# HiLab-git/FPL-plus

Hardware: AMD Instinct MI355X
Metric: 3D volumes/sec (train step, 80x160x160) (higher is better)
Workload: dtype bf16; 1 GPU; UNet3D-DSBN 32-base-ch bf16 (fp32 master weights), per-GPU batch 2x1x80x160x160 synthetic VS crops, DiceLoss + Adam, domain alternating per step; global_batch=2, parallelism=dp1, step=zero_grad+forward+loss+backward+allreduce+adam

## Files before the change

### fpl-plus_amd/csrc/elementwise.hip

```cpp
#include "common.h"
#include "philox.h"

namespace {

constexpr int EW_THREADS = 256;

template <typename T> struct Vec;
template <> struct Vec<float> {
  static constexpr int N = 4;
  typedef float4 raw;
  static __device__ __forceinline__ void load(const float* p, float (&v)[4]) {
    const float4 r = *reinterpret_cast<const float4*>(p);
    v[0] = r.x; v[1] = r.y; v[2] = r.z; v[3] = r.w;
  }
  static __device__ __forceinline__ void load_nt(const float* p, float (&v)[4]) { load(p, v); }
  static __device__ __forceinline__ void store(float* p, const float (&v)[4]) {
    *reinterpret_cast<float4*>(p) = make_float4(v[0], v[1], v[2], v[3]);
  }
};
template <> struct Vec<bf16_t> {
  static constexpr int N = 8;
  typedef __attribute__((ext_vector_type(8))) __bf16 raw;
  static __device__ __forceinline__ void load(const bf16_t* p, float (&v)[8]) {
    const raw r = *reinterpret_cast<const raw*>(p);
// ... 563 lines not shown
      vis[t] = ((n * D + pd * d_o + (t >> 2)) * H + 2 * ho + ((t >> 1) & 1)) * W + 2 * wo + (t & 1);
      ldv_nt<T, VEC>(y + vis[t] * ldy + c0, a[t]);
    }
#pragma unroll
    for (int j = 0; j < VEC; ++j) best[j] = -INFINITY;
#pragma unroll
    for (int t = 0; t < 8; ++t) {
      if (t >= 4 * pd) break;
#pragma unroll
      for (int j = 0; j < VEC; ++j) {
        float z = fmaf(a[t][j], sc[j], sh[j]);
        z = z > 0.f ? z : z * slope;
        z = (float)(T)z;
        a[t][j] = z;
        best[j] = z > best[j] ? z : best[j];
      }
      stv<T, VEC>(out + vis[t] * ldo + c0, a[t]);
    }
    stv<T, VEC>(pooled + vo * ldp + c0, best);
  }
}

template <typename T, int VEC>
__global__ void __launch_bounds__(EW_THREADS)
pool_bwd_bn_reduce_k(const T* __restrict__ y, int64_t ldy, const T* __restrict__ dy, int64_t lddy, const T* __restrict__ dskip,
                     int64_t lds, T* __restrict__ dx, int64_t ldo, const float* __restrict__ mean,
                     const float* __restrict__ rstd, const float* __restrict__ scale, const float* __restrict__ shift,
                     const float* __restrict__ slope_p, int N, int D, int H, int W, int C, int pd, float* __restrict__ part) {
  const int G = C / VEC, VL = EW_THREADS / G;
  const int g = threadIdx.x % G, vl = threadIdx.x / G, c0 = g * VEC;
  const int Do = D / pd, Ho = H / 2, Wo = W / 2;
  const int64_t vout = (int64_t)N * Do * Ho * Wo;
  const float slope = *slope_p;
  float sdz[VEC], sdx[VEC], sds = 0.f, m[VEC], rs[VEC], sc[VEC], sh[VEC];
#pragma unroll
  for (int j = 0; j < VEC; ++j) {
    sdz[j] = sdx[j] = 0.f;
    m[j] = mean[c0 + j]; rs[j] = rstd[c0 + j]; sc[j] = scale[c0 + j]; sh[j] = shift[c0 + j];
  }
  for (int64_t vo = (int64_t)blockIdx.x * VL + vl; vo < vout; vo += (int64_t)gridDim.x * VL) {
    int64_t q = vo;
    const int wo = (int)(q % Wo); q /= Wo;
    const int ho = (int)(q % Ho); q /= Ho;
    const int d_o = (int)(q % Do);
    const int64_t n = q / Do;
    float gr[VEC], best[VEC], a[8][VEC], o[8][VEC];
    int arg[VEC];
    int64_t vis[8];
    ldv<T, VEC>(dy + vo * lddy + c0, gr);
#pragma unroll
    for (int t = 0; t < 8; ++t) {
      if (t >= 4 * pd) break;
      vis[t] = ((n * D + pd * d_o + (t >> 2)) * H + 2 * ho + ((t >> 1) & 1)) * W + 2 * wo + (t & 1);
      ldv<T, VEC>(y + vis[t] * ldy + c0, a[t]);
      if (dskip) ldv<T, VEC>(dskip + vis[t] * lds + c0, o[t]);
      else {
#pragma unroll
        for (int j = 0; j < VEC; ++j) o[t][j] = 0.f;
      }
    }
#pragma unroll
    for (int j = 0; j < VEC; ++j) { best[j] = -INFINITY; arg[j] = 0; }
#pragma unroll
    for (int t = 0; t < 8; ++t) {
      if (t >= 4 * pd) break;
#pragma unroll
      for (int j = 0; j < VEC; ++j) {
        float z = fmaf(a[t][j], sc[j], sh[j]);
        z = z > 0.f ? z : z * slope;
        z = (float)(T)z;
        if (z > best[j]) { best[j] = z; arg[j] = t; }
      }
    }
#pragma unroll
    for (int t = 0; t < 8; ++t) {
      if (t >= 4 * pd) break;
#pragma unroll
      for (int j = 0; j < VEC; ++j) {
        const float dv = (float)(T)(o[t][j] + ((arg[j] == t) ? gr[j] : 0.f));
        o[t][j] = dv;
        const float z = fmaf(a[t][j], sc[j], sh[j]);
        const float dz = z > 0.f ? dv : dv * slope;
        sds += z > 0.f ? 0.f : dv * z;
        sdz[j] += dz;
        sdx[j] = fmaf(dz, (a[t][j] - m[j]) * rs[j], sdx[j]);
      }
      stv<T, VEC>(dx + vis[t] * ldo + c0, o[t]);
    }
  }
  __shared__ float red[EW_THREADS / 64 * 64][2 * VEC + 1];
  float* row = part + (int64_t)blockIdx.x * (2 * C + 1);
  for (int ofs = G; ofs < 64; ofs <<= 1) {
#pragma unroll
    for (int j = 0; j < VEC; ++j) { sdz[j] += __shfl_xor(sdz[j], ofs, 64); sdx[j] += __shfl_xor(sdx[j], ofs, 64); }
    sds += __shfl_xor(sds, ofs, 64);
  }
  const int lane = threadIdx.x & 63, wave = threadIdx.x >> 6;
  if (lane < G) {
#pragma unroll
    for (int j = 0; j < VEC; ++j) { red[wave * 64 + lane][j] = sdz[j]; red[wave * 64 + lane][VEC + j] = sdx[j]; }
    red[wave * 64 + lane][2 * VEC] = sds;
  }
  __syncthreads();
  if ((int)threadIdx.x < G) {
#pragma unroll
    for (int j = 0; j < VEC; ++j) {
      float t0 = 0.f, t1 = 0.f;
#pragma unroll
      for (int wv = 0; wv < EW_THREADS / 64; ++wv) { t0 += red[wv * 64 + threadIdx.x][j]; t1 += red[wv * 64 + threadIdx.x][VEC + j]; }
      row[c0 + j] = t0;
// ... 40 lines not shown
#pragma unroll
    for (int t = 0; t < 4; ++t) {
      if (t >= 2 * pd) break;
#pragma unroll
      for (int j = 0; j < VEC; ++j) {
        float z = fmaf(a[t][j], sc[j], sh[j]);
        z = z > 0.f ? z : z * slope;
        z = (float)(T)z;
        a[t][j] = z;
        best[j] = z > best[j] ? z : best[j];
      }
      stv<T, VEC>(out + vis[t] * ldo + c0, a[t]);
    }
#pragma unroll
    for (int j = 0; j < VEC; ++j) {
      const float o = __shfl_xor(best[j], G, 64);
      best[j] = o > best[j] ? o : best[j];
    }
    if (!(w & 1)) stv<T, VEC>(pooled + (int64_t)(u >> 1) * ldp + c0, best);
  }
}

template <typename T, int VEC>
__global__ void __launch_bounds__(EW_THREADS)
pool_bwd_bn_reduce_col_k(const T* __restrict__ y, int64_t ldy, const T* __restrict__ dy, int64_t lddy,
                         const T* __restrict__ dskip, int64_t lds, T* __restrict__ dx, int64_t ldo,
                         const float* __restrict__ mean, const float* __restrict__ rstd, const float* __restrict__ scale,
                         const float* __restrict__ shift, const float* __restrict__ slope_p, int N, int D, int H, int W, int C,
                         int pd, float* __restrict__ part) {
  const int G = C / VEC, VL = EW_THREADS / G;
  const int g = threadIdx.x % G, vl = threadIdx.x / G, c0 = g * VEC;
  const int Do = D / pd, Ho = H / 2;
  const unsigned units = (unsigned)N * Do * Ho * W;
  const float slope = *slope_p;
  float sdz[VEC], sdx[VEC], sds = 0.f, m[VEC], rs[VEC], sc[VEC], sh[VEC];
#pragma unroll
  for (int j = 0; j < VEC; ++j) {
    sdz[j] = sdx[j] = 0.f;
    m[j] = mean[c0 + j]; rs[j] = rstd[c0 + j]; sc[j] = scale[c0 + j]; sh[j] = shift[c0 + j];
  }
  for (unsigned u = blockIdx.x * VL + vl; u < units; u += gridDim.x * VL) {
    unsigned q = u;
    const int w = (int)(q % (unsigned)W); q /= (unsigned)W;
    const int ho = (int)(q % (unsigned)Ho); q /= (unsigned)Ho;
    const int d_o = (int)(q % (unsigned)Do);
    const int64_t n = q / (unsigned)Do;
    float gr[VEC], best[VEC], a[4][VEC], o[4][VEC];
    int arg[VEC];
    int64_t vis[4];
    ldv<T, VEC>(dy + (int64_t)(u >> 1) * lddy + c0, gr);
#pragma unroll
    for (int t = 0; t < 4; ++t) {
      if (t >= 2 * pd) break;
      vis[t] = ((n * D + pd * d_o + (t >> 1)) * H + 2 * ho + (t & 1)) * W + w;
      ldv<T, VEC>(y + vis[t] * ldy + c0, a[t]);
      if (dskip) ldv<T, VEC>(dskip + vis[t] * lds + c0, o[t]);
      else {
#pragma unroll
        for (int j = 0; j < VEC; ++j) o[t][j] = 0.f;
      }
    }
#pragma unroll
    for (int j = 0; j < VEC; ++j) { best[j] = -INFINITY; arg[j] = 8; }
#pragma unroll
    for (int t = 0; t < 4; ++t) {
      if (t >= 2 * pd) break;
#pragma unroll
      for (int j = 0; j < VEC; ++j) {
        float z = fmaf(a[t][j], sc[j], sh[j]);
        z = z > 0.f ? z : z * slope;
        z = (float)(T)z;
        if (z > best[j]) { best[j] = z; arg[j] = 2 * t + (w & 1); }
      }
    }
#pragma unroll
    for (int j = 0; j < VEC; ++j) {
      const float ob = __shfl_xor(best[j], G, 64);
      const int oa = __shfl_xor(arg[j], G, 64);
      if (ob > best[j] || (ob == best[j] && oa < arg[j])) arg[j] = -1;
    }
#pragma unroll
    for (int t = 0; t < 4; ++t) {
      if (t >= 2 * pd) break;
#pragma unroll
      for (int j = 0; j < VEC; ++j) {
        const float dv = (float)(T)(o[t][j] + ((arg[j] == 2 * t + (w & 1)) ? gr[j] : 0.f));
        o[t][j] = dv;
        const float z = fmaf(a[t][j], sc[j], sh[j]);
        const float dz = z > 0.f ? dv : dv * slope;
        sds += z > 0.f ? 0.f : dv * z;
        sdz[j] += dz;
        sdx[j] = fmaf(dz, (a[t][j] - m[j]) * rs[j], sdx[j]);
      }
      stv<T, VEC>(dx + vis[t] * ldo + c0, o[t]);
    }
  }
  __shared__ float red[EW_THREADS / 64 * 64][2 * VEC + 1];
  float* row = part + (int64_t)blockIdx.x * (2 * C + 1);
  for (int ofs = G; ofs < 64; ofs <<= 1) {
#pragma unroll
    for (int j = 0; j < VEC; ++j) { sdz[j] += __shfl_xor(sdz[j], ofs, 64); sdx[j] += __shfl_xor(sdx[j], ofs, 64); }
    sds += __shfl_xor(sds, ofs, 64);
  }
  const int lane = threadIdx.x & 63, wave = threadIdx.x >> 6;
  if (lane < G) {
#pragma unroll
    for (int j = 0; j < VEC; ++j) { red[wave * 64 + lane][j] = sdz[j]; red[wave * 64 + lane][VEC + j] = sdx[j]; }
    red[wave * 64 + lane][2 * VEC] = sds;
  }
  __syncthreads();
  if ((int)threadIdx.x < G) {
#pragma unroll
    for (int j = 0; j < VEC; ++j) {
      float t0 = 0.f, t1 = 0.f;
#pragma unroll
      for (int wv = 0; wv < EW_THREADS / 64; ++wv) { t0 += red[wv * 64 + threadIdx.x][j]; t1 += red[wv * 64 + threadIdx.x][VEC + j]; }
      row[c0 + j] = t0;
      row[C + c0 + j] = t1;
    }
  }
  if (threadIdx.x == 0) {
    float t = 0.f;
    for (int wv = 0; wv < EW_THREADS / 64; ++wv)
      for (int k = 0; k < G; ++k) t += red[wv * 64 + k][2 * VEC];
    row[2 * C] = t;
  }
}

__global__ void __launch_bounds__(EW_THREADS)
adam_k(float* __restrict__ p, const float* __restrict__ g, float* __restrict__ m, float* __restrict__ v, int64_t n,
       float step_size, float b1, float b2, float eps, float wd, float inv_sqrt_bc2, float gscale) {
  const FplxAdamConst c = {step_size, b1, b2, eps, wd, inv_sqrt_bc2, gscale, 1.f - b1, 1.f - b2};
  for (int64_t i = (int64_t)blockIdx.x * EW_THREADS + threadIdx.x; i < n; i += (int64_t)gridDim.x * EW_THREADS) {
    float pi = p[i], mi = m[i], vi = v[i];
    fplx_adam_elem(pi, g[i], mi, vi, c);
    m[i] = mi;
    v[i] = vi;
    p[i] = pi;
  }
}


template <typename T>
__global__ void __launch_bounds__(EW_THREADS)
channel_stats_k(const T* __restrict__ x, int64_t ld, int64_t V, int C, float* __restrict__ part) {
  const int c = blockIdx.y * 64 + (threadIdx.x & 63);
  const int vl = threadIdx.x >> 6;
  float s = 0.f, q = 0.f;
// ... 251 lines not shown
  FPLX_REQUIRE(n > 0 && c > 0 && d >= pd && h >= 2 && w >= 2 && !(d % pd) && !(h & 1) && !(w & 1) && (pd == 1 || pd == 2),
               FPLX_E_BADSHAPE, "%s: bad shape", what);
  FPLX_REQUIRE(fplx_bn_pool_fused_ok(c, dt), FPLX_E_BADSHAPE, "%s: C=%d dtype %d not supported (fplx_bn_pool_fused_ok)", what, c, dt);
  return FPLX_OK;
}

int fplx_bn_act_pool_fwd(const void* y, int64_t ldy, void* out, int64_t ldo, void* pooled, int64_t ldp, const float* scale,
                         const float* shift, const float* slope, int n, int d, int h, int w, int c, int dt, int pd,
                         fplx_stream_t stream) {
  FPLX_REQUIRE(y && out && pooled && scale && shift && slope, FPLX_E_NULL, "bn_act_pool_fwd: null pointer");
  const int rc = bn_pool_args_ok("bn_act_pool_fwd", n, d, h, w, c, dt, pd);
  if (rc != FPLX_OK) return rc;
  FPLX_REQUIRE(vec_ok<bf16_t>(y, ldy, out, ldo, pooled, ldp, c), FPLX_E_BADSHAPE, "bn_act_pool_fwd: pointers / leading dimensions not 16-byte aligned");
  const int64_t vo = (int64_t)n * (d / pd) * (h / 2) * (w / 2);
  if (fplx_knob(FPLX_K_POOL_COL) && c / 8 <= 32 && 2 * vo < ((int64_t)1 << 31))
    bn_act_pool_fwd_col_k<bf16_t, 8><<<ew_grid(2 * vo * (c / 8)), EW_THREADS, 0, (hipStream_t)stream>>>(
        (const bf16_t*)y, ldy, (bf16_t*)out, ldo, (bf16_t*)pooled, ldp, scale, shift, slope, n, d, h, w, c, pd);
  else
  bn_act_pool_fwd_k<bf16_t, 8><<<ew_grid(vo * (c / 8)), EW_THREADS, 0, (hipStream_t)stream>>>(
      (const bf16_t*)y, ldy, (bf16_t*)out, ldo, (bf16_t*)pooled, ldp, scale, shift, slope, n, d, h, w, c, pd);
  return fplx_check_launch("bn_act_pool_fwd");
}

int fplx_pool_bwd_bn_reduce(const void* y, int64_t ldy, const void* dy, int64_t lddy, const void* dskip, int64_t lds, void* dx,
                            int64_t ldo, const float* mean, const float* rstd, const float* scale, const float* shift,
                            const float* slope, int n, int d, int h, int w, int c, int dt, int pd, float* part,
                            fplx_stream_t stream) {
  FPLX_REQUIRE(y && dy && dx && mean && rstd && scale && shift && slope && part, FPLX_E_NULL, "pool_bwd_bn_reduce: null pointer");
  const int rc = bn_pool_args_ok("pool_bwd_bn_reduce", n, d, h, w, c, dt, pd);
  if (rc != FPLX_OK) return rc;
  FPLX_REQUIRE(vec_ok<bf16_t>(y, ldy, dy, lddy, dx, ldo, c) && vec_ok<bf16_t>(dskip, lds, nullptr, 0, nullptr, 0, c), FPLX_E_BADSHAPE,
               "pool_bwd_bn_reduce: pointers / leading dimensions not 16-byte aligned");
  const int rows = fplx_rows_for((int64_t)n * d * h * w);
  if (fplx_knob(FPLX_K_POOL_COL) && c / 8 <= 32 && (int64_t)n * (d / pd) * (h / 2) * w < ((int64_t)1 << 31))
    pool_bwd_bn_reduce_col_k<bf16_t, 8><<<rows, EW_THREADS, 0, (hipStream_t)stream>>>(
        (const bf16_t*)y, ldy, (const bf16_t*)dy, lddy, (const bf16_t*)dskip, lds, (bf16_t*)dx, ldo, mean, rstd, scale, shift, slope, n,
        d, h, w, c, pd, part);
  else
  pool_bwd_bn_reduce_k<bf16_t, 8><<<rows, EW_THREADS, 0, (hipStream_t)stream>>>(
      (const bf16_t*)y, ldy, (const bf16_t*)dy, lddy, (const bf16_t*)dskip, lds, (bf16_t*)dx, ldo, mean, rstd, scale, shift, slope, n,
      d, h, w, c, pd, part);
  return fplx_check_launch("pool_bwd_bn_reduce");
}

int fplx_adam_step(float* p, const float* g, float* m, float* v, int64_t n, float lr, float beta1, float beta2,
                   float eps, float weight_decay, int step, float grad_scale, fplx_stream_t stream) {
  FPLX_REQUIRE(p && g && m && v, FPLX_E_NULL, "adam_step: null pointer");
  FPLX_REQUIRE(n > 0 && step >= 1, FPLX_E_BADSHAPE, "adam_step: n=%lld step=%d", (long long)n, step);
  const double bc1 = 1.0 - pow((double)beta1, step), bc2 = 1.0 - pow((double)beta2, step);
  adam_k<<<ew_grid(n), EW_THREADS, 0, (hipStream_t)stream>>>(p, g, m, v, n, (float)((double)lr / bc1), beta1, beta2, eps,
                                                            weight_decay, (float)(1.0 / sqrt(bc2)), grad_scale);
  return fplx_check_launch("adam_step");
}

}
```

### fpl-plus_amd/fplx/_lib.py

```python
import ctypes
import os
import re

_RUNTIME_ENV = (("GPU_MAX_HW_QUEUES", "8"), ("HIP_FORCE_DEV_KERNARG", "1"))
_env_preset = {k: os.environ.get(k) for k, _ in _RUNTIME_ENV}
for _k, _v in _RUNTIME_ENV:
    os.environ.setdefault(_k, _v)

import torch


def runtime_env_report():
    return dict(_env_report)


_gpu_was_up = bool(torch.cuda.is_initialized())
_env_report = {}
for _k, _v in _RUNTIME_ENV:
    _env_report[_k] = (os.environ.get(_k), "preset" if _env_preset[_k] is not None else ("too late" if _gpu_was_up else "fplx"))
_late = [k for k, (_, how) in _env_report.items() if how == "too late"]
if _late:
    import warnings
    warnings.warn(
        "fplx was imported after the GPU had been initialised and %s %s not in the environment: the HIP runtime reads %s only "
# ... 98 lines not shown
    try:
        while _lib.fplx_tuning_key(i, buf, 64) >= 0:
            key = buf.value.decode()
            env = os.environ.get("FPLX_" + key.upper())
            if env is not None:
                try:
                    val = int(env)
                except ValueError:
                    raise ValueError("fplx: FPLX_%s=%r is not an integer" % (key.upper(), env))
                rc = _lib.fplx_set_tuning(key.encode(), val)
                if rc != 0:
                    raise FplxError("fplx (%d): fplx_set_tuning(%s, %d) failed" % (rc, key, val))
            i += 1
    except Exception:
        _lib = None
        raise


_HOST_KNOBS = {
    "pack_reuse": 1,
    "side_stream": 1,
    "split_cat": 1,
    "fused_pool": 1,
    "eval_fuse": 1,
    "stem_wg_main": 1,
    "outconv_fuse": 1,
    "stem_wgrad_bn": 1,
    "outconv_wgrad_bn": 1,
    "bucket_elems": 1 << 21,
    "pack_small_multi": 1,
    "adam_pack": 1,
    "ddp_overlap_all": 1,
}
_host_vals = {}


def host_knob(key):
    if key not in _HOST_KNOBS:
        raise ValueError("fplx: unknown host knob %r" % (key,))
    if key not in _host_vals:
        env = os.environ.get("FPLX_" + key.upper())
        try:
            _host_vals[key] = _HOST_KNOBS[key] if env is None else int(env)
        except ValueError:
            raise ValueError("fplx: FPLX_%s=%r is not an integer" % (key.upper(), env))
    return _host_vals[key]
# ... 20 lines not shown
```

### fpl-plus_amd/fplx/engine.py

```python

import torch
from . import ops, _lib
from ._lib import F32, BF16

LEVEL_OF_BLOCK = [0, 1, 2, 3, 4, 3, 2, 1, 0]


class Saved(object):
    __slots__ = ("x", "dims", "domain", "train", "seed", "step", "blocks", "cats", "pooled", "packs",
                 "drop_on", "deconv_in", "skips", "split", "oc_fused", "oc_wg", "pack_gen")


class Engine(object):
    def __init__(self, net):
        self.net = net
        self.ws = None
        self.ws_side = None
        self._pack_cache = None
        self._train_packs = None
        self._pack_bufs = None
        self._adam_packs = None
        self._pack_gen = 0
        self.use_adam_pack = _lib.host_knob("adam_pack") != 0
        self.use_pack_multi = _lib.host_knob("pack_small_multi") != 0
        self.allow_pack_reuse = _lib.host_knob("pack_reuse") != 0
        self._side = None
        self.use_side_stream = _lib.host_knob("side_stream") != 0
        self.use_split_cat = _lib.host_knob("split_cat") != 0
        self.use_fused_pool = _lib.host_knob("fused_pool") != 0
        self.use_eval_fusion = _lib.host_knob("eval_fuse") != 0
        self.stem_wgrad_on_main = _lib.host_knob("stem_wg_main") != 0
        self.use_outconv_fusion = _lib.host_knob("outconv_fuse") != 0
        self.use_stem_wgrad_bn = _lib.host_knob("stem_wgrad_bn") != 0
        self.use_outconv_wgrad_bn = _lib.host_knob("outconv_wgrad_bn") != 0
        self._fold_cache = {}
        self.defer_probe = False
        self._deferred = []
        self.block_joins = None
        self.debug_tap = None

    def _workspace(self, nbytes, dev):
        if self.ws is None or self.ws.numel() < nbytes or self.ws.device != dev:
            self.ws = torch.empty(int(nbytes), dtype=torch.uint8, device=dev)
            self.ws_side = torch.empty(int(nbytes), dtype=torch.uint8, device=dev)
        return self.ws

    def _persistent_packs(self, act_dtype):
        net = self.net
        if not self.use_adam_pack or act_dtype != torch.bfloat16:
            return {}
        dev = net.flat_params.device
        if self._pack_bufs is None or self._pack_bufs[0] != act_dtype or self._pack_bufs[1] != dev:
# ... 443 lines not shown
            end = (o + n + 3) // 4 * 4
            pending = getattr(getattr(on_ready, "__self__", None), "pending", None)
            if pending is not None and not pending(end):
                return
            if side_on and pending is not None and not block_joins:
                ev = torch.cuda.Event()
                ev.record(main)
                side.wait_event(ev)
                with torch.cuda.stream(side):
                    on_ready(end)
                return
            join_side()
            on_ready(end)

        d_cur = empty(vox[0], ft[0])
        oc_fused = bool(sv.oc_fused)
        if not oc_fused:
            ops.conv3d_fwd(dlogits, ops.planar_strides(ncls, D, H, W), F32, packs["out_conv"][1], None, d_cur,
                           ops.cl_strides(D, H, W, ft[0]), a_dt, dims[0], ncls, ft[0], (1, 3, 3), None)
        outconv_wgrad()
        ready("out_conv.bias")

        def site_bwd(key, bnkey, relukey, y, bnbuf, p, sid, d_out, xin, xs, x_dt, cin, l, want_dx, dx_view, reduced=False,
                     wgrad_here=False, from_logits=False):
            c = ft[l]
            gkey = "%s.bns.%d" % (bnkey, domain)
            if from_logits:
                ops.outconv_dgrad_bn_bwd(dlogits, packs["out_conv"][1], y, bnbuf, net.get_param(relukey + ".weight"), sv.train,
                                         gv[gkey + ".weight"], gv[gkey + ".bias"], gv[relukey + ".weight"], part, coef, d_out,
                                         dims[l], c, ncls)
            else:
                stem_fused = (self.use_stem_wgrad_bn and not want_dx and tap is None and sv.train and x_dt == F32 and p == 0.0 and
                              gv[key + ".weight"].dim() == 5 and adt == torch.bfloat16 and not isinstance(xin, tuple) and
                              ops.ld_of(d_out) % 8 == 0 and d_out.data_ptr() % 16 == 0 and ops.stem_wgrad_bn_ok(dims[l], cin, c))
                ops.bn_act_bwd(y, d_out, d_out, bnbuf, net.get_param(relukey + ".weight"), p, sv.seed, sid, c, sv.train,
                               gv[gkey + ".weight"], gv[gkey + ".bias"], gv[relukey + ".weight"], part, coef, reduced,
                               apply=not stem_fused)
                if stem_fused:
                    fn = lambda: ops.stem_wgrad_bn(xin, y, d_out, bnbuf, net.get_param(relukey + ".weight"), coef,
                                                   gv[key + ".weight"], dims[l], cin, c, ws if wgrad_here else ws_w)
                    if wgrad_here:
                        fn()
                    else:
                        on_side(fn, d_out, xin, y, coef)
                    return
            if tap is not None:
                tap(key + ".dy", d_out)
            db = None if sv.train else gv[key + ".bias"]
            gw = gv[key + ".weight"]
            two_d = gw.dim() == 4
            if isinstance(xin, tuple):
                if want_dx:
                    ops.conv3d_dgrad_split2(d_out, packs[key][1], dx_view[0], dx_view[1], dims[l], cin, c, two_d)
                    if tap is not None:
                        tap(key + ".dx0", dx_view[0])
                        tap(key + ".dx1", dx_view[1])
                on_side(lambda: ops.conv3d_wgrad_cat2(xin[0], xin[1], d_out, gw, dims[l], cin, c, ws_w, two_d),
                        d_out, xin[0], xin[1])
                return
            def wg():
                if wgrad_here:
                    fn = ops.conv2d_wgrad if two_d else ops.conv3d_wgrad
                    args = (xin, xs, x_dt, d_out, ops.cl_strides(*dims[l][1:], c), a_dt, gw, db, dims[l], cin, c)
                    fn(*(args + ((ws,) if two_d else ((3, 3, 3), ws))))
                elif two_d:
                    on_side(lambda: ops.conv2d_wgrad(xin, xs, x_dt, d_out, ops.cl_strides(*dims[l][1:], c), a_dt, gw, db,
                                                     dims[l], cin, c, ws_w), d_out, xin)
                else:
                    on_side(lambda: ops.conv3d_wgrad(xin, xs, x_dt, d_out, ops.cl_strides(*dims[l][1:], c), a_dt, gw, db,
                                                     dims[l], cin, c, (3, 3, 3), ws_w), d_out, xin)
            if want_dx:
                ops.conv3d_fwd(d_out, ops.cl_strides(*dims[l][1:], c), a_dt, packs[key][1], None, dx_view,
                               ops.cl_strides(*dims[l][1:], ops.ld_of(dx_view)), a_dt, dims[l], c, cin, (3, 3, 3), None,
                               mid=two_d)
                if tap is not None:
                    tap(key + ".dx", dx_view)
            wg()

        def block_bwd(b, d_out, want_dx, reduced=False):
            blk = sv.blocks[b]
            key = net.block_keys[b]
            mod = net.block_modules[b]
            l, c, cin = blk["l"], ft[blk["l"]], blk["cin"]
            d_a1 = empty(vox[l], c)
            site_bwd(key + "." + mod.cname(2), key + "." + mod.bname(2), key + ".relu_2", blk["y2"], blk["bn2"], 0.0, 0,
                     d_out, blk["a1"], ops.cl_strides(*dims[l][1:], c), a_dt, c, l, True, d_a1, reduced,
                     from_logits=(b == 8 and oc_fused))
            if isinstance(blk["xin"], tuple):
                d_in = (empty(vox[l], cin // 2), empty(vox[l], cin // 2)) if want_dx else None
            else:
                d_in = empty(vox[l], cin) if want_dx else None
            site_bwd(key + "." + mod.cname(1), key + "." + mod.bname(1), key + ".relu_1", blk["y1"], blk["bn1"], blk["p1"],
                     blk["sid"], d_a1, blk["xin"], blk["xs"], blk["x_dt"], cin, l, want_dx, d_in,
                     wgrad_here=(b == 0 and side_on and self.stem_wgrad_on_main))
            return d_in

        d_skips = [None] * 4
        for j in range(3, -1, -1):
            l = 3 - j
            d_cat = block_bwd(5 + j, d_cur, True)
            if isinstance(d_cat, tuple):
                d_skips[l], d_up = d_cat
            else:
                d_skips[l] = d_cat[:, :ft[l]]
                d_up = d_cat[:, ft[l]:]
            name = "up%d.%s" % (j + 1, net.up_modules[j].tname())
            xin = sv.deconv_in[j]
            if net.bilinear:
                d_low = empty(vox[l + 1], ft[l])
                ops.upsample2_bwd(d_up, d_low, dims[l + 1], ft[l], pds[l])
# ... 3 lines not shown
                    ft[l], (1, 1, 1), ws_w), d_low, d_up, d_cat, xin)
                ready(name + ".bias")
                d_cur = empty(vox[l + 1], ft[l + 1])
                ops.conv3d_fwd(d_low, lows, a_dt, packs[name][1], None, d_cur, highs, a_dt, dims[l + 1], ft[l], ft[l + 1],
                               (1, 1, 1), None)
                if tap is not None:
                    tap(name + ".dx", d_cur)
                continue
            def deconv_wgrad(xin=xin, d_up=d_up, name=name, l=l, d_cat=d_cat):
                on_side(lambda: ops.deconv2_wgrad(xin, d_up, gv[name + ".weight"], gv[name + ".bias"], dims[l + 1], ft[l + 1],
                                                  ft[l], ws_w, pds[l]), d_up, d_cat, xin)
            d_cur = empty(vox[l + 1], ft[l + 1])
            ops.deconv2_dgrad(d_up, packs[name][1], d_cur, dims[l + 1], ft[l + 1], ft[l], pds[l])
            deconv_wgrad()
            ready(name + ".bias")
            if tap is not None:
                tap(name + ".dx", d_cur)
        decoder_phase[0] = False
        d_pool = block_bwd(4, d_cur, True)
        ready("block4.conv.relu_1.weight")
        for i in range(3, -1, -1):
            d_a2 = empty(vox[i], ft[i])
            fused = self.use_fused_pool and ops.bn_pool_fused_ok(ft[i], adt)
            if fused:
                blk = sv.blocks[i]
                ops.pool_bwd_bn_reduce(blk["y2"], d_pool, d_skips[i], d_a2, blk["bn2"],
                                       net.get_param(net.block_keys[i] + ".relu_2.weight"), dims[i], ft[i], part, pds[i])
            else:
                ops.maxpool2_bwd(sv.skips[i], d_pool, d_skips[i], d_a2, dims[i], ft[i], pds[i])
            d_pool = block_bwd(i, d_a2, i > 0, fused)
            ready("block%d.conv.relu_1.weight" % i)
        join_side()
        del keep
        return gflat
```

### fpl-plus_amd/fplx/ops.py

```python
import ctypes
import math

import numpy as np
import torch
from . import _lib
from ._lib import F32, BF16, call

_DT = {torch.float32: F32, torch.bfloat16: BF16}


def dt_of(t):
    try:
        return _DT[t.dtype]
    except KeyError:
        raise ValueError("fplx: unsupported activation dtype {0:}".format(t.dtype))


def ptr(t):
    return 0 if t is None else t.data_ptr()


def stream():
    return torch.cuda.current_stream().cuda_stream

# ... 278 lines not shown
        raise ValueError("fplx: partial-row buffer too small for the fused out_conv backward (%d < %d floats)" % (part.numel(), rows * (2 * c0 + 1)))
    bn = [ptr(bnbuf[0]), ptr(bnbuf[1]), ptr(bnbuf[2]), ptr(bnbuf[3])]
    call("fplx_outconv_dgrad_bn_reduce", ptr(dlogits), ptr(wb), ptr(y), ld_of(y), bn[0], bn[1], bn[2], bn[3], ptr(slope), ptr(part),
         n, d, h, w, int(c0), int(ncls), stream())
    call("fplx_bn_act_bwd_finalize", ptr(part), rows, int(c0), y.shape[0], 1 if train else 0, ptr(dgamma), ptr(dbeta), ptr(dslope),
         ptr(coef), stream())
    call("fplx_outconv_dgrad_bn_apply", ptr(dlogits), ptr(wb), ptr(y), ld_of(y), bn[0], bn[1], bn[2], bn[3], ptr(slope), ptr(coef),
         ptr(dy), ld_of(dy), n, d, h, w, int(c0), int(ncls), stream())


def bn_pool_fused_ok(c, dtype):
    return _lib.lib().fplx_bn_pool_fused_ok(int(c), _DT[dtype]) == 1


def bn_act_pool_fwd(y, out, pooled, bnbuf, slope, dims, c, pd=2):
    n, d, h, w = dims
    call("fplx_bn_act_pool_fwd", ptr(y), ld_of(y), ptr(out), ld_of(out), ptr(pooled), ld_of(pooled), ptr(bnbuf[2]), ptr(bnbuf[3]),
         ptr(slope), n, d, h, w, c, dt_of(y), pd, stream())


def pool_bwd_bn_reduce(y, dy, dskip, dx, bnbuf, slope, dims, c, part, pd=2):
    n, d, h, w = dims
    call("fplx_pool_bwd_bn_reduce", ptr(y), ld_of(y), ptr(dy), ld_of(dy), ptr(dskip), 0 if dskip is None else ld_of(dskip), ptr(dx),
         ld_of(dx), ptr(bnbuf[0]), ptr(bnbuf[1]), ptr(bnbuf[2]), ptr(bnbuf[3]), ptr(slope), n, d, h, w, c, dt_of(y), pd, ptr(part),
         stream())


def bn_act_bwd(y, dout, dy, bnbuf, slope, p, seed, sid, c, train, dgamma, dbeta, dslope, part, coef, reduced=False, apply=True):
    v = y.shape[0]
    rows = num_partials(v)
    if not reduced:
        call("fplx_bn_act_bwd_reduce", ptr(y), ld_of(y), ptr(dout), ld_of(dout), ptr(bnbuf[0]), ptr(bnbuf[1]),
             ptr(bnbuf[2]), ptr(bnbuf[3]), ptr(slope), float(p), int(seed), int(sid), v, c, dt_of(y), ptr(part), stream())
    call("fplx_bn_act_bwd_finalize", ptr(part), rows, c, v, 1 if train else 0, ptr(dgamma), ptr(dbeta), ptr(dslope),
         ptr(coef), stream())
    if not apply:
        return
    call("fplx_bn_act_bwd_apply", ptr(y), ld_of(y), ptr(dout), ld_of(dout), ptr(dy), ld_of(dy), ptr(bnbuf[0]),
         ptr(bnbuf[1]), ptr(bnbuf[2]), ptr(bnbuf[3]), ptr(slope), ptr(coef), float(p), int(seed), int(sid), v, c,
         dt_of(y), stream())


def stem_wgrad_bn_ok(dims, cin, cout):
    import ctypes
    n, d, h, w = dims
    kern, g, ks, r = ctypes.c_int(), ctypes.c_int(), ctypes.c_int(), ctypes.c_int()
    _lib.check(_lib.lib().fplx_conv3d_plan_query(n, d, h, w, int(cin), int(cout), 3, 3, 3, F32, BF16, ctypes.byref(kern),
# ... 469 lines not shown
```

### include/fplx.h

```cpp
#ifndef FPLX_H
#define FPLX_H

#include <stddef.h>
#include <stdint.h>

#ifdef __cplusplus
extern "C" {
#endif
#pragma GCC visibility push(default)

typedef void* fplx_stream_t;

enum { FPLX_F32 = 0, FPLX_BF16 = 1 };

enum {
  FPLX_OK = 0,
  FPLX_E_BADSHAPE = -1,
  FPLX_E_BADDTYPE = -2,
  FPLX_E_WORKSPACE = -3,
  FPLX_E_HIP = -4,
  FPLX_E_NULL = -5
};

int fplx_version(void);
// ... 109 lines not shown
                           const float* mean, const float* rstd, const float* scale, const float* shift,
                           const float* slope, float p, uint64_t seed, uint32_t stream_id,
                           int64_t voxels, int c, int dt, float* part, fplx_stream_t stream);
int fplx_bn_act_bwd_finalize(const float* part, int rows, int c, int64_t count, int train,
                             float* dgamma, float* dbeta, float* dslope, float* coef, fplx_stream_t stream);
int fplx_bn_act_bwd_apply(const void* y, int64_t ldy, const void* dout, int64_t ldd, void* dy, int64_t ldo,
                          const float* mean, const float* rstd, const float* scale, const float* shift,
                          const float* slope, const float* coef, float p, uint64_t seed, uint32_t stream_id,
                          int64_t voxels, int c, int dt, fplx_stream_t stream);

int fplx_maxpool2_fwd(const void* x, int64_t ldx, void* y, int64_t ldy, int n, int d, int h, int w, int c,
                      int dt, fplx_stream_t stream);
int fplx_maxpool2_bwd(const void* x, int64_t ldx, const void* dy, int64_t ldy, const void* dskip, int64_t lds,
                      void* dx, int64_t ldo, int n, int d, int h, int w, int c, int dt, fplx_stream_t stream);

int fplx_bn_pool_fused_ok(int c, int dt);
int fplx_bn_act_pool_fwd(const void* y, int64_t ldy, void* out, int64_t ldo, void* pooled, int64_t ldp, const float* scale,
                         const float* shift, const float* slope, int n, int d, int h, int w, int c, int dt, int pd,
                         fplx_stream_t stream);
int fplx_pool_bwd_bn_reduce(const void* y, int64_t ldy, const void* dy, int64_t lddy, const void* dskip, int64_t lds, void* dx,
                            int64_t ldo, const float* mean, const float* rstd, const float* scale, const float* shift,
                            const float* slope, int n, int d, int h, int w, int c, int dt, int pd, float* part,
                            fplx_stream_t stream);

int fplx_outconv_bn_rows(int n, int d, int h, int w, int c0, int ncls);
int fplx_outconv_fwd_bn(const void* y, int64_t ldy, const float* scale, const float* shift, const float* prelu_slope, void* a,
                        int64_t lda, const float* wf, const float* bias, float* logits, int n, int d, int h, int w, int c0,
                        int ncls, fplx_stream_t stream);
int fplx_outconv_dgrad_bn_reduce(const float* dlogits, const void* wb, const void* y, int64_t ldy, const float* mean,
                                 const float* rstd, const float* scale, const float* shift, const float* prelu_slope,
                                 float* part, int n, int d, int h, int w, int c0, int ncls, fplx_stream_t stream);
int fplx_outconv_dgrad_bn_apply(const float* dlogits, const void* wb, const void* y, int64_t ldy, const float* mean,
                                const float* rstd, const float* scale, const float* shift, const float* prelu_slope,
                                const float* coef, void* dy, int64_t lddy, int n, int d, int h, int w, int c0, int ncls,
                                fplx_stream_t stream);
size_t fplx_outconv_wgrad_bn_ws_bytes(int n, int d, int h, int w, int c0, int ncls);
int fplx_outconv_wgrad_bn(const void* y, int64_t ldy, const float* scale, const float* shift, const float* prelu_slope,
                          const float* dlogits, float* dw, float* db, int n, int d, int h, int w, int c0, int ncls, void* ws,
                          size_t ws_bytes, fplx_stream_t stream);

int fplx_upsample2_fwd(const void* x, int64_t ldx, void* y, int64_t ldy, int n, int d, int h, int w, int c, int dt, int sd,
                       fplx_stream_t stream);
int fplx_upsample2_bwd(const void* dy, int64_t ldy, void* dx, int64_t ldx, int n, int d, int h, int w, int c, int dt, int sd,
                       fplx_stream_t stream);

#define FPLX_LOSS_K(C) (6 * (C) + 3)
// ... 101 lines not shown
```

Measured before the change: 252.2 volumes/s.

## Recompute pooled gradient in BN apply pass instead of materializing it

In the encoder backward pass, the fused pool-backward + BN-reduce kernel no longer writes the unpooled gradient tensor when the new knob is on. A new pool_bwd_bn_apply kernel recomputes the max-pool argmax and skip-gradient sum from y, dy and dskip, then applies the BN/PReLU backward coefficients directly. This replaces a full-size bf16 write and its later read with re-reads of y, dy and dskip plus some recomputation. The intent is to cut memory traffic on the largest encoder activations.

```diff
diff --git a/fpl-plus_amd/csrc/elementwise.hip b/fpl-plus_amd/csrc/elementwise.hip
--- a/fpl-plus_amd/csrc/elementwise.hip
+++ b/fpl-plus_amd/csrc/elementwise.hip
@@ -609,6 +609,25 @@
 }
 
 template <typename T, int VEC>
+__device__ __forceinline__ void pool_window_arg(const float (&a)[8][VEC], const float (&sc)[VEC], const float (&sh)[VEC],
+                                                float slope, int pd, int (&arg)[VEC]) {
+  float best[VEC];
+#pragma unroll
+  for (int j = 0; j < VEC; ++j) { best[j] = -INFINITY; arg[j] = 0; }
+#pragma unroll
+  for (int t = 0; t < 8; ++t) {
+    if (t >= 4 * pd) break;
+#pragma unroll
+    for (int j = 0; j < VEC; ++j) {
+      float z = fmaf(a[t][j], sc[j], sh[j]);
+      z = z > 0.f ? z : z * slope;
+      z = (float)(T)z;
+      if (z > best[j]) { best[j] = z; arg[j] = t; }
+    }
+  }
+}
+
+template <typename T, int VEC, bool STORE = true>
 __global__ void __launch_bounds__(EW_THREADS)
 pool_bwd_bn_reduce_k(const T* __restrict__ y, int64_t ldy, const T* __restrict__ dy, int64_t lddy, const T* __restrict__ dskip,
                      int64_t lds, T* __restrict__ dx, int64_t ldo, const float* __restrict__ mean,
@@ -631,7 +650,7 @@
     const int ho = (int)(q % Ho); q /= Ho;
     const int d_o = (int)(q % Do);
     const int64_t n = q / Do;
-    float gr[VEC], best[VEC], a[8][VEC], o[8][VEC];
+    float gr[VEC], a[8][VEC], o[8][VEC];
     int arg[VEC];
     int64_t vis[8];
     ldv<T, VEC>(dy + vo * lddy + c0, gr);
@@ -646,19 +665,7 @@
         for (int j = 0; j < VEC; ++j) o[t][j] = 0.f;
       }
     }
-#pragma unroll
-    for (int j = 0; j < VEC; ++j) { best[j] = -INFINITY; arg[j] = 0; }
-#pragma unroll
-    for (int t = 0; t < 8; ++t) {
-      if (t >= 4 * pd) break;
-#pragma unroll
-      for (int j = 0; j < VEC; ++j) {
-        float z = fmaf(a[t][j], sc[j], sh[j]);
-        z = z > 0.f ? z : z * slope;
-        z = (float)(T)z;
-        if (z > best[j]) { best[j] = z; arg[j] = t; }
-      }
-    }
+    pool_window_arg<T, VEC>(a, sc, sh, slope, pd, arg);
 #pragma unroll
     for (int t = 0; t < 8; ++t) {
       if (t >= 4 * pd) break;
@@ -672,7 +679,7 @@
         sdz[j] += dz;
         sdx[j] = fmaf(dz, (a[t][j] - m[j]) * rs[j], sdx[j]);
       }
-      stv<T, VEC>(dx + vis[t] * ldo + c0, o[t]);
+      if constexpr (STORE) stv<T, VEC>(dx + vis[t] * ldo + c0, o[t]);
     }
   }
   __shared__ float red[EW_THREADS / 64 * 64][2 * VEC + 1];
@@ -759,6 +766,31 @@
 }
 
 template <typename T, int VEC>
+__device__ __forceinline__ void pool_column_arg(const float (&a)[4][VEC], const float (&sc)[VEC], const float (&sh)[VEC],
+                                                float slope, int pd, int w, int G, int (&arg)[VEC]) {
+  float best[VEC];
+#pragma unroll
+  for (int j = 0; j < VEC; ++j) { best[j] = -INFINITY; arg[j] = 8; }
+#pragma unroll
+  for (int t = 0; t < 4; ++t) {
+    if (t >= 2 * pd) break;
+#pragma unroll
+    for (int j = 0; j < VEC; ++j) {
+      float z = fmaf(a[t][j], sc[j], sh[j]);
+      z = z > 0.f ? z : z * slope;
+      z = (float)(T)z;
+      if (z > best[j]) { best[j] = z; arg[j] = 2 * t + (w & 1); }
+    }
+  }
+#pragma unroll
+  for (int j = 0; j < VEC; ++j) {
+    const float ob = __shfl_xor(best[j], G, 64);
+    const int oa = __shfl_xor(arg[j], G, 64);
+    if (ob > best[j] || (ob == best[j] && oa < arg[j])) arg[j] = -1;
+  }
+}
+
+template <typename T, int VEC, bool STORE = true>
 __global__ void __launch_bounds__(EW_THREADS)
 pool_bwd_bn_reduce_col_k(const T* __restrict__ y, int64_t ldy, const T* __restrict__ dy, int64_t lddy,
                          const T* __restrict__ dskip, int64_t lds, T* __restrict__ dx, int64_t ldo,
@@ -782,7 +814,7 @@
     const int ho = (int)(q % (unsigned)Ho); q /= (unsigned)Ho;
     const int d_o = (int)(q % (unsigned)Do);
     const int64_t n = q / (unsigned)Do;
-    float gr[VEC], best[VEC], a[4][VEC], o[4][VEC];
+    float gr[VEC], a[4][VEC], o[4][VEC];
     int arg[VEC];
     int64_t vis[4];
     ldv<T, VEC>(dy + (int64_t)(u >> 1) * lddy + c0, gr);
@@ -797,25 +829,7 @@
         for (int j = 0; j < VEC; ++j) o[t][j] = 0.f;
       }
     }
-#pragma unroll
-    for (int j = 0; j < VEC; ++j) { best[j] = -INFINITY; arg[j] = 8; }
-#pragma unroll
-    for (int t = 0; t < 4; ++t) {
-      if (t >= 2 * pd) break;
-#pragma unroll
-      for (int j = 0; j < VEC; ++j) {
-        float z = fmaf(a[t][j], sc[j], sh[j]);
-        z = z > 0.f ? z : z * slope;
-        z = (float)(T)z;
-        if (z > best[j]) { best[j] = z; arg[j] = 2 * t + (w & 1); }
-      }
-    }
-#pragma unroll
-    for (int j = 0; j < VEC; ++j) {
-      const float ob = __shfl_xor(best[j], G, 64);
-      const int oa = __shfl_xor(arg[j], G, 64);
-      if (ob > best[j] || (ob == best[j] && oa < arg[j])) arg[j] = -1;
-    }
+    pool_column_arg<T, VEC>(a, sc, sh, slope, pd, w, G, arg);
 #pragma unroll
     for (int t = 0; t < 4; ++t) {
       if (t >= 2 * pd) break;
@@ -829,7 +843,7 @@
         sdz[j] += dz;
         sdx[j] = fmaf(dz, (a[t][j] - m[j]) * rs[j], sdx[j]);
       }
-      stv<T, VEC>(dx + vis[t] * ldo + c0, o[t]);
+      if constexpr (STORE) stv<T, VEC>(dx + vis[t] * ldo + c0, o[t]);
     }
   }
   __shared__ float red[EW_THREADS / 64 * 64][2 * VEC + 1];
@@ -861,6 +875,117 @@
     for (int wv = 0; wv < EW_THREADS / 64; ++wv)
       for (int k = 0; k < G; ++k) t += red[wv * 64 + k][2 * VEC];
     row[2 * C] = t;
+  }
+}
+
+template <typename T, int VEC>
+__global__ void __launch_bounds__(EW_THREADS)
+pool_bwd_bn_apply_k(const T* __restrict__ y, int64_t ldy, const T* __restrict__ dy, int64_t lddy, const T* __restrict__ dskip,
+                    int64_t lds, T* __restrict__ dx, int64_t ldo, const float* __restrict__ mean, const float* __restrict__ rstd,
+                    const float* __restrict__ scale, const float* __restrict__ shift, const float* __restrict__ slope_p,
+                    const float* __restrict__ coef, int N, int D, int H, int W, int C, int pd) {
+  const int G = C / VEC, VL = EW_THREADS / G;
+  const int g = threadIdx.x % G, vl = threadIdx.x / G, c0 = g * VEC;
+  const int Do = D / pd, Ho = H / 2, Wo = W / 2;
+  const int64_t vout = (int64_t)N * Do * Ho * Wo;
+  const float slope = *slope_p;
+  float m[VEC], rs[VEC], sc[VEC], sh[VEC], k0[VEC], k1[VEC];
+#pragma unroll
+  for (int j = 0; j < VEC; ++j) {
+    m[j] = mean[c0 + j]; rs[j] = rstd[c0 + j]; sc[j] = scale[c0 + j]; sh[j] = shift[c0 + j];
+    k0[j] = coef[c0 + j]; k1[j] = coef[C + c0 + j];
+  }
+  for (int64_t vo = (int64_t)blockIdx.x * VL + vl; vo < vout; vo += (int64_t)gridDim.x * VL) {
+    int64_t q = vo;
+    const int wo = (int)(q % Wo); q /= Wo;
+    const int ho = (int)(q % Ho); q /= Ho;
+    const int d_o = (int)(q % Do);
+    const int64_t n = q / Do;
+    float gr[VEC], a[8][VEC], o[8][VEC];
+    int arg[VEC];
+    int64_t vis[8];
+    ldv_nt<T, VEC>(dy + vo * lddy + c0, gr);
+#pragma unroll
+    for (int t = 0; t < 8; ++t) {
+      if (t >= 4 * pd) break;
+      vis[t] = ((n * D + pd * d_o + (t >> 2)) * H + 2 * ho + ((t >> 1) & 1)) * W + 2 * wo + (t & 1);
+      ldv_nt<T, VEC>(y + vis[t] * ldy + c0, a[t]);
+      if (dskip) ldv_nt<T, VEC>(dskip + vis[t] * lds + c0, o[t]);
+      else {
+#pragma unroll
+        for (int j = 0; j < VEC; ++j) o[t][j] = 0.f;
+      }
+    }
+    pool_window_arg<T, VEC>(a, sc, sh, slope, pd, arg);
+#pragma unroll
+    for (int t = 0; t < 8; ++t) {
+      if (t >= 4 * pd) break;
+#pragma unroll
+      for (int j = 0; j < VEC; ++j) {
+        const float dv = (float)(T)(o[t][j] + ((arg[j] == t) ? gr[j] : 0.f));
+        const float z = fmaf(a[t][j], sc[j], sh[j]);
+        const float dz = z > 0.f ? dv : dv * slope;
+        const float xh = (a[t][j] - m[j]) * rs[j];
+        o[t][j] = sc[j] * (dz - k0[j] - xh * k1[j]);
+      }
+      stv<T, VEC>(dx + vis[t] * ldo + c0, o[t]);
+    }
+  }
+}
+
+template <typename T, int VEC>
+__global__ void __launch_bounds__(EW_THREADS)
+pool_bwd_bn_apply_col_k(const T* __restrict__ y, int64_t ldy, const T* __restrict__ dy, int64_t lddy,
+                        const T* __restrict__ dskip, int64_t lds, T* __restrict__ dx, int64_t ldo,
+                        const float* __restrict__ mean, const float* __restrict__ rstd, const float* __restrict__ scale,
+                        const float* __restrict__ shift, const float* __restrict__ slope_p, const float* __restrict__ coef,
+                        int N, int D, int H, int W, int C, int pd) {
+  const int G = C / VEC, VL = EW_THREADS / G;
+  const int g = threadIdx.x % G, vl = threadIdx.x / G, c0 = g * VEC;
+  const int Do = D / pd, Ho = H / 2;
+  const unsigned units = (unsigned)N * Do * Ho * W;
+  const float slope = *slope_p;
+  float m[VEC], rs[VEC], sc[VEC], sh[VEC], k0[VEC], k1[VEC];
+#pragma unroll
+  for (int j = 0; j < VEC; ++j) {
+    m[j] = mean[c0 + j]; rs[j] = rstd[c0 + j]; sc[j] = scale[c0 + j]; sh[j] = shift[c0 + j];
+    k0[j] = coef[c0 + j]; k1[j] = coef[C + c0 + j];
+  }
+  for (unsigned u = blockIdx.x * VL + vl; u < units; u += gridDim.x * VL) {
+    unsigned q = u;
+    const int w = (int)(q % (unsigned)W); q /= (unsigned)W;
+    const int ho = (int)(q % (unsigned)Ho); q /= (unsigned)Ho;
+    const int d_o = (int)(q % (unsigned)Do);
+    const int64_t n = q / (unsigned)Do;
+    float gr[VEC], a[4][VEC], o[4][VEC];
+    int arg[VEC];
+    int64_t vis[4];
+    ldv_nt<T, VEC>(dy + (int64_t)(u >> 1) * lddy + c0, gr);
+#pragma unroll
+    for (int t = 0; t < 4; ++t) {
+      if (t >= 2 * pd) break;
+      vis[t] = ((n * D + pd * d_o + (t >> 1)) * H + 2 * ho + (t & 1)) * W + w;
+      ldv_nt<T, VEC>(y + vis[t] * ldy + c0, a[t]);
+      if (dskip) ldv_nt<T, VEC>(dskip + vis[t] * lds + c0, o[t]);
+      else {
+#pragma unroll
+        for (int j = 0; j < VEC; ++j) o[t][j] = 0.f;
+      }
+    }
+    pool_column_arg<T, VEC>(a, sc, sh, slope, pd, w, G, arg);
+#pragma unroll
+    for (int t = 0; t < 4; ++t) {
+      if (t >= 2 * pd) break;
+#pragma unroll
+      for (int j = 0; j < VEC; ++j) {
+        const float dv = (float)(T)(o[t][j] + ((arg[j] == 2 * t + (w & 1)) ? gr[j] : 0.f));
+        const float z = fmaf(a[t][j], sc[j], sh[j]);
+        const float dz = z > 0.f ? dv : dv * slope;
+        const float xh = (a[t][j] - m[j]) * rs[j];
+        o[t][j] = sc[j] * (dz - k0[j] - xh * k1[j]);
+      }
+      stv<T, VEC>(dx + vis[t] * ldo + c0, o[t]);
+    }
   }
 }
 
@@ -1158,25 +1283,49 @@
   return fplx_check_launch("bn_act_pool_fwd");
 }
 
+static bool pool_col_form(int n, int d, int h, int w, int c, int pd) {
+  return fplx_knob(FPLX_K_POOL_COL) && c / 8 <= 32 && (int64_t)n * (d / pd) * (h / 2) * w < ((int64_t)1 << 31);
+}
+
 int fplx_pool_bwd_bn_reduce(const void* y, int64_t ldy, const void* dy, int64_t lddy, const void* dskip, int64_t lds, void* dx,
                             int64_t ldo, const float* mean, const float* rstd, const float* scale, const float* shift,
                             const float* slope, int n, int d, int h, int w, int c, int dt, int pd, float* part,
                             fplx_stream_t stream) {
-  FPLX_REQUIRE(y && dy && dx && mean && rstd && scale && shift && slope && part, FPLX_E_NULL, "pool_bwd_bn_reduce: null pointer");
+  FPLX_REQUIRE(y && dy && mean && rstd && scale && shift && slope && part, FPLX_E_NULL, "pool_bwd_bn_reduce: null pointer");
   const int rc = bn_pool_args_ok("pool_bwd_bn_reduce", n, d, h, w, c, dt, pd);
   if (rc != FPLX_OK) return rc;
   FPLX_REQUIRE(vec_ok<bf16_t>(y, ldy, dy, lddy, dx, ldo, c) && vec_ok<bf16_t>(dskip, lds, nullptr, 0, nullptr, 0, c), FPLX_E_BADSHAPE,
                "pool_bwd_bn_reduce: pointers / leading dimensions not 16-byte aligned");
   const int rows = fplx_rows_for((int64_t)n * d * h * w);
-  if (fplx_knob(FPLX_K_POOL_COL) && c / 8 <= 32 && (int64_t)n * (d / pd) * (h / 2) * w < ((int64_t)1 << 31))
-    pool_bwd_bn_reduce_col_k<bf16_t, 8><<<rows, EW_THREADS, 0, (hipStream_t)stream>>>(
-        (const bf16_t*)y, ldy, (const bf16_t*)dy, lddy, (const bf16_t*)dskip, lds, (bf16_t*)dx, ldo, mean, rstd, scale, shift, slope, n,
-        d, h, w, c, pd, part);
+#define POOL_REDUCE(K_, S_) K_<bf16_t, 8, S_><<<rows, EW_THREADS, 0, (hipStream_t)stream>>>(                                       \
+      (const bf16_t*)y, ldy, (const bf16_t*)dy, lddy, (const bf16_t*)dskip, lds, (bf16_t*)dx, ldo, mean, rstd, scale, shift, slope, n, \
+      d, h, w, c, pd, part)
+  if (pool_col_form(n, d, h, w, c, pd)) { if (dx) POOL_REDUCE(pool_bwd_bn_reduce_col_k, true); else POOL_REDUCE(pool_bwd_bn_reduce_col_k, false); }
+  else if (dx) POOL_REDUCE(pool_bwd_bn_reduce_k, true);
+  else POOL_REDUCE(pool_bwd_bn_reduce_k, false);
+#undef POOL_REDUCE
+  return fplx_check_launch("pool_bwd_bn_reduce");
+}
+
+int fplx_pool_bwd_bn_apply(const void* y, int64_t ldy, const void* dy, int64_t lddy, const void* dskip, int64_t lds, void* dx,
+                           int64_t ldo, const float* mean, const float* rstd, const float* scale, const float* shift,
+                           const float* slope, const float* coef, int n, int d, int h, int w, int c, int dt, int pd,
+                           fplx_stream_t stream) {
+  FPLX_REQUIRE(y && dy && dx && mean && rstd && scale && shift && slope && coef, FPLX_E_NULL, "pool_bwd_bn_apply: null pointer");
+  const int rc = bn_pool_args_ok("pool_bwd_bn_apply", n, d, h, w, c, dt, pd);
+  if (rc != FPLX_OK) return rc;
+  FPLX_REQUIRE(vec_ok<bf16_t>(y, ldy, dy, lddy, dx, ldo, c) && vec_ok<bf16_t>(dskip, lds, nullptr, 0, nullptr, 0, c), FPLX_E_BADSHAPE,
+               "pool_bwd_bn_apply: pointers / leading dimensions not 16-byte aligned");
+  const int64_t vo = (int64_t)n * (d / pd) * (h / 2) * (w / 2);
+  if (pool_col_form(n, d, h, w, c, pd))
+    pool_bwd_bn_apply_col_k<bf16_t, 8><<<ew_grid(2 * vo * (c / 8)), EW_THREADS, 0, (hipStream_t)stream>>>(
+        (const bf16_t*)y, ldy, (const bf16_t*)dy, lddy, (const bf16_t*)dskip, lds, (bf16_t*)dx, ldo, mean, rstd, scale, shift, slope,
+        coef, n, d, h, w, c, pd);
   else
-  pool_bwd_bn_reduce_k<bf16_t, 8><<<rows, EW_THREADS, 0, (hipStream_t)stream>>>(
-      (const bf16_t*)y, ldy, (const bf16_t*)dy, lddy, (const bf16_t*)dskip, lds, (bf16_t*)dx, ldo, mean, rstd, scale, shift, slope, n,
-      d, h, w, c, pd, part);
-  return fplx_check_launch("pool_bwd_bn_reduce");
+    pool_bwd_bn_apply_k<bf16_t, 8><<<ew_grid(vo * (c / 8)), EW_THREADS, 0, (hipStream_t)stream>>>(
+        (const bf16_t*)y, ldy, (const bf16_t*)dy, lddy, (const bf16_t*)dskip, lds, (bf16_t*)dx, ldo, mean, rstd, scale, shift, slope,
+        coef, n, d, h, w, c, pd);
+  return fplx_check_launch("pool_bwd_bn_apply");
 }
 
 int fplx_adam_step(float* p, const float* g, float* m, float* v, int64_t n, float lr, float beta1, float beta2,
diff --git a/fpl-plus_amd/fplx/_lib.py b/fpl-plus_amd/fplx/_lib.py
--- a/fpl-plus_amd/fplx/_lib.py
+++ b/fpl-plus_amd/fplx/_lib.py
@@ -144,6 +144,7 @@
     "side_stream": 1,
     "split_cat": 1,
     "fused_pool": 1,
+    "pool_bwd_apply": 1,
     "eval_fuse": 1,
     "stem_wg_main": 1,
     "outconv_fuse": 1,
diff --git a/fpl-plus_amd/fplx/engine.py b/fpl-plus_amd/fplx/engine.py
--- a/fpl-plus_amd/fplx/engine.py
+++ b/fpl-plus_amd/fplx/engine.py
@@ -28,6 +28,7 @@
         self.use_side_stream = _lib.host_knob("side_stream") != 0
         self.use_split_cat = _lib.host_knob("split_cat") != 0
         self.use_fused_pool = _lib.host_knob("fused_pool") != 0
+        self.use_pool_bwd_apply = _lib.host_knob("pool_bwd_apply") != 0
         self.use_eval_fusion = _lib.host_knob("eval_fuse") != 0
         self.stem_wgrad_on_main = _lib.host_knob("stem_wg_main") != 0
         self.use_outconv_fusion = _lib.host_knob("outconv_fuse") != 0
@@ -517,7 +518,7 @@
         ready("out_conv.bias")
 
         def site_bwd(key, bnkey, relukey, y, bnbuf, p, sid, d_out, xin, xs, x_dt, cin, l, want_dx, dx_view, reduced=False,
-                     wgrad_here=False, from_logits=False):
+                     wgrad_here=False, from_logits=False, pool=None):
             c = ft[l]
             gkey = "%s.bns.%d" % (bnkey, domain)
             if from_logits:
@@ -530,7 +531,10 @@
                               ops.ld_of(d_out) % 8 == 0 and d_out.data_ptr() % 16 == 0 and ops.stem_wgrad_bn_ok(dims[l], cin, c))
                 ops.bn_act_bwd(y, d_out, d_out, bnbuf, net.get_param(relukey + ".weight"), p, sv.seed, sid, c, sv.train,
                                gv[gkey + ".weight"], gv[gkey + ".bias"], gv[relukey + ".weight"], part, coef, reduced,
-                               apply=not stem_fused)
+                               apply=not stem_fused and pool is None)
+                if pool is not None:
+                    ops.pool_bwd_bn_apply(y, pool[0], pool[1], d_out, bnbuf, net.get_param(relukey + ".weight"), coef, dims[l], c,
+                                          pds[l])
                 if stem_fused:
                     fn = lambda: ops.stem_wgrad_bn(xin, y, d_out, bnbuf, net.get_param(relukey + ".weight"), coef,
                                                    gv[key + ".weight"], dims[l], cin, c, ws if wgrad_here else ws_w)
@@ -572,7 +576,7 @@
                     tap(key + ".dx", dx_view)
             wg()
 
-        def block_bwd(b, d_out, want_dx, reduced=False):
+        def block_bwd(b, d_out, want_dx, reduced=False, pool=None):
             blk = sv.blocks[b]
             key = net.block_keys[b]
             mod = net.block_modules[b]
@@ -580,7 +584,7 @@
             d_a1 = empty(vox[l], c)
             site_bwd(key + "." + mod.cname(2), key + "." + mod.bname(2), key + ".relu_2", blk["y2"], blk["bn2"], 0.0, 0,
                      d_out, blk["a1"], ops.cl_strides(*dims[l][1:], c), a_dt, c, l, True, d_a1, reduced,
-                     from_logits=(b == 8 and oc_fused))
+                     from_logits=(b == 8 and oc_fused), pool=pool)
             if isinstance(blk["xin"], tuple):
                 d_in = (empty(vox[l], cin // 2), empty(vox[l], cin // 2)) if want_dx else None
             else:
@@ -630,13 +634,14 @@
         for i in range(3, -1, -1):
             d_a2 = empty(vox[i], ft[i])
             fused = self.use_fused_pool and ops.bn_pool_fused_ok(ft[i], adt)
+            pool = (d_pool, d_skips[i]) if fused and self.use_pool_bwd_apply else None
             if fused:
                 blk = sv.blocks[i]
-                ops.pool_bwd_bn_reduce(blk["y2"], d_pool, d_skips[i], d_a2, blk["bn2"],
+                ops.pool_bwd_bn_reduce(blk["y2"], d_pool, d_skips[i], None if pool else d_a2, blk["bn2"],
                                        net.get_param(net.block_keys[i] + ".relu_2.weight"), dims[i], ft[i], part, pds[i])
             else:
                 ops.maxpool2_bwd(sv.skips[i], d_pool, d_skips[i], d_a2, dims[i], ft[i], pds[i])
-            d_pool = block_bwd(i, d_a2, i > 0, fused)
+            d_pool = block_bwd(i, d_a2, i > 0, fused, pool)
             ready("block%d.conv.relu_1.weight" % i)
         join_side()
         del keep
diff --git a/fpl-plus_amd/fplx/ops.py b/fpl-plus_amd/fplx/ops.py
--- a/fpl-plus_amd/fplx/ops.py
+++ b/fpl-plus_amd/fplx/ops.py
@@ -324,7 +324,14 @@
 def pool_bwd_bn_reduce(y, dy, dskip, dx, bnbuf, slope, dims, c, part, pd=2):
     n, d, h, w = dims
     call("fplx_pool_bwd_bn_reduce", ptr(y), ld_of(y), ptr(dy), ld_of(dy), ptr(dskip), 0 if dskip is None else ld_of(dskip), ptr(dx),
-         ld_of(dx), ptr(bnbuf[0]), ptr(bnbuf[1]), ptr(bnbuf[2]), ptr(bnbuf[3]), ptr(slope), n, d, h, w, c, dt_of(y), pd, ptr(part),
+         c if dx is None else ld_of(dx), ptr(bnbuf[0]), ptr(bnbuf[1]), ptr(bnbuf[2]), ptr(bnbuf[3]), ptr(slope), n, d, h, w, c,
+         dt_of(y), pd, ptr(part), stream())
+
+
+def pool_bwd_bn_apply(y, dy, dskip, dx, bnbuf, slope, coef, dims, c, pd=2):
+    n, d, h, w = dims
+    call("fplx_pool_bwd_bn_apply", ptr(y), ld_of(y), ptr(dy), ld_of(dy), ptr(dskip), 0 if dskip is None else ld_of(dskip), ptr(dx),
+         ld_of(dx), ptr(bnbuf[0]), ptr(bnbuf[1]), ptr(bnbuf[2]), ptr(bnbuf[3]), ptr(slope), ptr(coef), n, d, h, w, c, dt_of(y), pd,
          stream())
 
 
diff --git a/include/fplx.h b/include/fplx.h
--- a/include/fplx.h
+++ b/include/fplx.h
@@ -155,6 +155,10 @@
                             int64_t ldo, const float* mean, const float* rstd, const float* scale, const float* shift,
                             const float* slope, int n, int d, int h, int w, int c, int dt, int pd, float* part,
                             fplx_stream_t stream);
+int fplx_pool_bwd_bn_apply(const void* y, int64_t ldy, const void* dy, int64_t lddy, const void* dskip, int64_t lds, void* dx,
+                           int64_t ldo, const float* mean, const float* rstd, const float* scale, const float* shift,
+                           const float* slope, const float* coef, int n, int d, int h, int w, int c, int dt, int pd,
+                           fplx_stream_t stream);
 
 int fplx_outconv_bn_rows(int n, int d, int h, int w, int c0, int ncls);
 int fplx_outconv_fwd_bn(const void* y, int64_t ldy, const float* scale, const float* shift, const float* prelu_slope, void* a,
```

Result: no change. 249.9 volumes/s (-0.9%).
